# rbrito/deprecated-lame-mirror

Hardware: AMD Instinct MI355X
Metric: encoded audio seconds/sec (x real-time) at 44.1kHz stereo CBR128 (higher is better)
Workload: dtype f32

## Files before the change

### deprecated-lame-mirror_amd/csrc/lh_analysis.hip

```cpp
#include <stdint.h>
#include <math.h>

#ifdef LH_EMU
#include "hipemu.h"
#define LH_CONST static const
#else
#include <hip/hip_runtime.h>
#define LH_CONST __device__ static const
#endif

#if defined(LH_APROF) && !defined(LH_EMU)
__shared__ unsigned long long *lh_ap_base;
#define LH_PT(var) unsigned long long var = clock64()
#define LH_PA(idx, var) do { if (c.lane == 0) atomicAdd(&lh_ap_base[LH_NPROF * c.wave + 20 + (idx)], clock64() - var); } while (0)
#define LH_PC(idx) do { } while (0)
#endif
#define LH_CUSTOM_LDS "lh_lds_analysis.h"
#define LH_CUSTOM_SMP
#define LH_FZ_X(i) ((((i) >> 4) & 2) | (((i) >> 3) & 24) | (((i) >> 5) & 4))
#define LH_FZ(i) ((i) ^ LH_FZ_X(i))
#define LH_STAGE_IDX(i) LH_FZ(i)
#include "lh_static_tables.h"
#include "lh_dev_common.h"
#if !defined(LH_EMU)
// ... 312 lines not shown
    int     al[4], ah[4];
    if (K1 == 4) {
        int const x = LH_FZ_X(lo);
#pragma unroll
        for (int j = 0; j < 4; j++) {
            al[j] = (lo + j * K1) ^ x;
            ah[j] = (hi + j * K1) ^ x;
        }
    }
    else if (K1 == 16) {
        int const x = LH_FZ_X(blk * k4);
#pragma unroll
        for (int j = 0; j < 4; j++) {
            al[j] = (lo + j * K1) ^ x ^ (j >= 2 ? 2 : 0);
            ah[j] = (hi + j * K1) ^ x ^ (j >= 2 ? 2 : 0);
        }
    }
    else if (K1 == 64) {
#pragma unroll
        for (int j = 0; j < 4; j++) {
            al[j] = (lo + j * K1) ^ LH_FZ_X(64 * j);
            ah[j] = (hi + j * K1) ^ (2 ^ LH_FZ_X(64 * j));
        }
    }
    else {
        int const xl = LH_FZ_X(lo), xh = LH_FZ_X(hi);
#pragma unroll
        for (int j = 0; j < 4; j++) {
            al[j] = (lo + j * K1) ^ xl;
            ah[j] = (hi + j * K1) ^ xh;
        }
    }
    float const p0 = fz[al[0]], p1 = fz[al[1]], p2 = fz[al[2]], p3 = fz[al[3]];
    float const q0 = fz[ah[0]], q1 = fz[ah[1]], q2 = fz[ah[2]], q3 = fz[ah[3]];
    float const s01 = p0 + p1, d01 = p0 - p1, s23 = p2 + p3, d23 = p2 - p3;
    float const r2 = (float) (LH_SQRT2 * q2), r3 = (float) (LH_SQRT2 * q3);
    float const t01 = q0 + q1, u01 = q0 - q1;
    float const a_l0 = s01 + s23, a_l1 = d01 + d23, a_l2 = s01 - s23, a_l3 = d01 - d23;
    float const a_h0 = t01 + r2, a_h1 = u01 + r3, a_h2 = t01 - r2, a_h3 = u01 - r3;
    LhRot const rq1 = lh_rot(tw.z, tw.w, p1, q1);
    LhRot const rq3 = lh_rot(tw.z, tw.w, p3, q3);
    float const le = p0 + rq1.along, lm = p0 - rq1.along;
    float const he = q0 + rq1.across, hm = q0 - rq1.across;
    float const l2e = p2 + rq3.along, l2m = p2 - rq3.along;
    float const h2e = q2 + rq3.across, h2m = q2 - rq3.across;
    LhRot const ra = lh_rot(tw.x, tw.y, l2e, h2m);
    LhRot const rb = lh_rot(tw.y, tw.x, h2e, l2m);
    fz[al[0]] = axis ? a_l0 : le + ra.along;
    fz[al[1]] = axis ? a_l1 : lm + rb.across;
    fz[al[2]] = axis ? a_l2 : le - ra.along;
    fz[al[3]] = axis ? a_l3 : lm - rb.across;
    fz[ah[0]] = axis ? a_h0 : he + rb.along;
    fz[ah[1]] = axis ? a_h1 : hm + ra.across;
    fz[ah[2]] = axis ? a_h2 : he - rb.along;
    fz[ah[3]] = axis ? a_h3 : hm - ra.across;
}

LH_DEVFN void
lh_fft_long_inplace(const LhCtx & c, float *x)
{
    const float *w = c.T->fft_window;
    int const lane = c.lane;
    float   o[2][8];
#pragma unroll
    for (int q = 0; q < 2; q++) {
        int const jj = lane + 64 * q;
        int const i = (int) lh_rev8((unsigned) jj);
        const float *xs = x + (i ^ LH_FZ_X(i));
        float   f0, f1, f2, f3, ww;
        f0 = w[i] * xs[0];
        ww = w[i + 0x200] * xs[0x200];
        f1 = f0 - ww;
        f0 = f0 + ww;
        f2 = w[i + 0x100] * xs[0x100];
        ww = w[i + 0x300] * xs[0x300];
        f3 = f2 - ww;
        f2 = f2 + ww;
        o[q][0] = f0 + f2;
        o[q][2] = f0 - f2;
        o[q][1] = f1 + f3;
        o[q][3] = f1 - f3;
        f0 = w[i + 0x001] * xs[0x001];
        ww = w[i + 0x201] * xs[0x201];
        f1 = f0 - ww;
        f0 = f0 + ww;
        f2 = w[i + 0x101] * xs[0x101];
        ww = w[i + 0x301] * xs[0x301];
        f3 = f2 - ww;
        f2 = f2 + ww;
        o[q][4] = f0 + f2;
        o[q][6] = f0 - f2;
        o[q][5] = f1 + f3;
        o[q][7] = f1 - f3;
    }
    {
        lh_f32x4 tw[4][2];
#pragma unroll
        for (int stage = 0; stage < 4; stage++) {
            int const kx = 2 << (2 * stage);
#pragma unroll
            for (int q = 0; q < 2; q++)
                tw[stage][q] = *(const lh_f32x4 *) c.T->fht_tw[stage][(lane + 64 * q) % kx];
        }
        LH_WAVE_SYNC_MEM();
#pragma unroll
        for (int q = 0; q < 2; q++) {
            int const at = 4 * (lane + 64 * q), xa = LH_FZ_X(at);
#pragma unroll
            for (int k = 0; k < 4; k++) {
                x[(at + k) ^ xa] = o[q][k];
                x[(at + k + LH_BLKSIZE / 2) ^ xa] = o[q][4 + k];
            }
        }
        LH_WAVE_SYNC_MEM();
#pragma unroll
        for (int q = 0; q < 2; q++)
            lh_fht_unit_fz < 4 > (tw[0][q], x, lane + 64 * q);
        LH_WAVE_SYNC_MEM();
#pragma unroll
        for (int q = 0; q < 2; q++)
            lh_fht_unit_fz < 16 > (tw[1][q], x, lane + 64 * q);
        LH_WAVE_SYNC_MEM();
#pragma unroll
        for (int q = 0; q < 2; q++)
            lh_fht_unit_fz < 64 > (tw[2][q], x, lane + 64 * q);
        LH_WAVE_SYNC_MEM();
#pragma unroll
        for (int q = 0; q < 2; q++)
            lh_fht_unit_fz < 256 > (tw[3][q], x, lane + 64 * q);
        LH_WAVE_SYNC_MEM();
    }
}

LH_DEVFN void
lh_fft_short_inplace(const LhCtx & c, float *x)
{
    const float *ws = c.T->fft_window_s;
    int const lane = c.lane;
    float   o[2][8];
#pragma unroll
    for (int q = 0; q < 2; q++) {
        int const t = lane + 64 * q, tt = t < 3 * (LH_BLKSIZE_S / 8) ? t : 0;
        int const b = tt >> 5, j = tt & 31;
        int const k = (576 / 3) * (b + 1);
        int const i = (int) lh_rev8((unsigned) (j << 2));
        float   f0, f1, f2, f3, w;
        f0 = ws[i] * x[LH_FZ(i + k)];
        w = ws[0x7f - i] * x[LH_FZ(i + k + 0x80)];
        f1 = f0 - w;
        f0 = f0 + w;
        f2 = ws[i + 0x40] * x[LH_FZ(i + k + 0x40)];
        w = ws[0x3f - i] * x[LH_FZ(i + k + 0xc0)];
        f3 = f2 - w;
        f2 = f2 + w;
        o[q][0] = f0 + f2;
        o[q][2] = f0 - f2;
        o[q][1] = f1 + f3;
        o[q][3] = f1 - f3;
        f0 = ws[i + 0x01] * x[LH_FZ(i + k + 0x01)];
        w = ws[0x7e - i] * x[LH_FZ(i + k + 0x81)];
        f1 = f0 - w;
        f0 = f0 + w;
        f2 = ws[i + 0x41] * x[LH_FZ(i + k + 0x41)];
        w = ws[0x3e - i] * x[LH_FZ(i + k + 0xc1)];
        f3 = f2 - w;
        f2 = f2 + w;
        o[q][4] = f0 + f2;
        o[q][6] = f0 - f2;
        o[q][5] = f1 + f3;
        o[q][7] = f1 - f3;
    }
    LH_WAVE_SYNC_MEM();
#pragma unroll
    for (int q = 0; q < 2; q++) {
        int const t = lane + 64 * q;
        if (t < 3 * (LH_BLKSIZE_S / 8)) {
            int const at = (t >> 5) * LH_BLKSIZE_S + 4 * (t & 31);
#pragma unroll
            for (int k = 0; k < 4; k++) {
                x[LH_FZ(at + k)] = o[q][k];
                x[LH_FZ(at + k + LH_BLKSIZE_S / 2)] = o[q][4 + k];
            }
        }
    }
    LH_WAVE_SYNC_MEM();
    for (int t = lane; t < 3 * (LH_BLKSIZE_S / 8); t += 64) {
        int const b = t >> 5, u = t & 31;
        lh_fht_unit_fz < 4 > (*(const lh_f32x4 *) c.T->fht_tw[0][u % 2], x + b * LH_BLKSIZE_S, u);
    }
    LH_WAVE_SYNC_MEM();
    for (int t = lane; t < 3 * (LH_BLKSIZE_S / 8); t += 64) {
        int const b = t >> 5, u = t & 31;
        lh_fht_unit_fz < 16 > (*(const lh_f32x4 *) c.T->fht_tw[1][u % 8], x + b * LH_BLKSIZE_S, u);
    }
    LH_WAVE_SYNC_MEM();
    for (int t = lane; t < 3 * (LH_BLKSIZE_S / 8); t += 64) {
        int const b = t >> 5, u = t & 31;
        lh_fht_unit_fz < 64 > (*(const lh_f32x4 *) c.T->fht_tw[2][u % 32], x + b * LH_BLKSIZE_S, u);
    }
    LH_WAVE_SYNC_MEM();
}

LH_DEVFN void
lh_an_spectra_short(const LhCtx & c, int w, int both, const float *wl, const float *wr, int first, float *out_own, float *out_ms)
{
    float const sqrt2_half = (float) (LH_SQRT2 * 0.5f);
    int const n = LH_BLKSIZE_S, h = n >> 1;
    for (int m = c.lane; m <= h; m += 64) {
        int const ire = first + m, iim = first + ((m == 0) ? 0 : (n - m));
        float const lre = wl[LH_FZ(ire)], lim = wl[LH_FZ(iim)], rre = wr[LH_FZ(ire)], rim = wr[LH_FZ(iim)];
        float const ore = w ? rre : lre, oim = w ? rim : lim;
        float const mre = (w ? lre - rre : lre + rre) * sqrt2_half, mim = (w ? lim - rim : lim + rim) * sqrt2_half;
        out_own[m] = (m == 0) ? ore * ore : (ore * ore + oim * oim) * 0.5f;
        if (both)
            out_ms[m] = (m == 0) ? mre * mre : (mre * mre + mim * mim) * 0.5f;
    }
}

LH_DEVFN void
lh_an_spectra(const LhCtx & c, int w, int own, int ms, float *work)
{
    float const sqrt2_half = (float) (LH_SQRT2 * 0.5f);
    const float *wl = work, *wr = work + LH_BLKSIZE;
    float   eo[9], em[9];
#pragma unroll
    for (int k = 0; k < 9; k++) {
        int const m0 = c.lane + 64 * k, m = m0 <= LH_BLKSIZE / 2 ? m0 : LH_BLKSIZE / 2;
        int const ire = m, iim = (m == 0) ? 0 : (LH_BLKSIZE - m);
        float const lre = wl[LH_FZ(ire)], lim = wl[LH_FZ(iim)], rre = wr[LH_FZ(ire)], rim = wr[LH_FZ(iim)];
        float const ore = w ? rre : lre, oim = w ? rim : lim;
        float const mre = (w ? lre - rre : lre + rre) * sqrt2_half, mim = (w ? lim - rim : lim + rim) * sqrt2_half;
        eo[k] = (m == 0) ? ore * ore : (ore * ore + oim * oim) * 0.5f;
        em[k] = (m == 0) ? mre * mre : (mre * mre + mim * mim) * 0.5f;
    }
    LH_SYNC_WG_LDS();
#pragma unroll
    for (int k = 0; k < 9; k++) {
        int const m = c.lane + 64 * k;
        if (m <= LH_BLKSIZE / 2) {
            if (own)
                work[w * LH_AN_ROW + m] = eo[k];
            if (ms)
                work[(w + 2) * LH_AN_ROW + m] = em[k];
        }
    }
}

#ifndef LH_EMU
extern "C" __global__ void __launch_bounds__(LH_NT, 6)
#else
void
#endif
lh_analysis_kernel(const LhConfig * LH_KRESTRICT cfg, const LhTables * LH_KRESTRICT T, const int16_t * LH_KRESTRICT pcm, const float *pcmf, const LhStreamDesc * descs,
                   LhMidFrame * frames, int nstreams, LhStreamState * states)
{
#if defined(LH_APROF) && !defined(LH_EMU)
    unsigned long long *aprof = &states[blockIdx.y].prof[0][0];
    if (threadIdx.x == 0)
        lh_ap_base = aprof;
#endif
    LH_AP_T0();
    LhLds & L = lh_lds;
    LhLds & P = L;
    float  *const work = L.work;
#define LH_AN_E(chn) (work + (chn) * LH_AN_ROW)
    int const sidx = (int) blockIdx.y;
    LhCtx   c;
    c.cfg = cfg;
    c.T = T;
    c.st = nullptr;
    c.pcm = pcm;
    c.pcmf = pcmf;
    c.d = lh_desc_uniform(descs, sidx);
    c.tid = (int) threadIdx.x;
    c.lane = c.tid & 63;
    c.wave = lh_uni_i(c.tid >> 6);
    LhGranuleAt const ga = lh_granule_at(c.d, (int) blockIdx.x);
    if (!ga.live)
        return;
    int const lane = c.lane, w = c.wave, gr = ga.gr;
    int const n_chn_psy = (cfg->mode == LH_MODE_JOINT_STEREO) ? 4 : cfg->channels;
    int const bufbase = 576 + gr * 576 - LH_FFTOFFSET;
    LhMidGr *mg = &frames[ga.at].small.gr[gr];
    if (c.tid < 2)
        L.uselong[c.tid] = mg->uselong[c.tid];
    LH_AP(0);
    lh_stage_span < LH_BLKSIZE, LH_NT > (c, LH_SPAN, LH_SPAN + LH_BLKSIZE, ga.frame_base + bufbase);
    LH_SYNC_WG_LDS();
    LH_AP(1);
    if (w < cfg->channels)
        lh_fft_long_inplace(c, work + w * LH_BLKSIZE);
    LH_SYNC_WG_LDS();
    LH_AP(2);
    lh_an_spectra(c, w, w < n_chn_psy, n_chn_psy == 4, work);
    LH_WAVE_SYNC_MEM();
    const float *stg_s3 = T->psy_l.s3;
    LH_WAVE_SYNC_MEM();
    LH_AP(3);
    LH_AP(4);
    {
        int const chn = (lane == 1) ? w + 2 : w;
        int const summing = lane < 3 && chn < n_chn_psy;
        int const loud = (lane == 2);
        float  *prod = (w == 0) ? P.eb : P.thr;
        const float *ew = T->ath_eql_w;
        const float *e = LH_AN_E(summing ? chn : w);
        float   acc = 0.0f;
        for (int h = 0; h < 2; h++) {
            int const j0 = 256 * h;
            LH_WAVE_SYNC_MEM();
#pragma unroll
            for (int q = 0; q < 4; q++) {
                int const j = j0 + lane + 64 * q;
                prod[j - j0] = LH_AN_E(w)[j] * ew[j];
            }
            LH_WAVE_SYNC_MEM();
            if (summing) {
                const lh_f32x4 *s4 = (const lh_f32x4 *) ((loud ? prod - j0 : e) + j0);
                lh_f32x4 a0 = s4[0], a1 = s4[1], a2 = s4[2], a3 = s4[3];
                if (h == 0 && !loud) {
                    a0.x = a0.y = a0.z = a0.w = 0.0f;
                    a1.x = a1.y = a1.z = a1.w = 0.0f;
                    a2.x = a2.y = a2.z = 0.0f;
                }
                for (int g = 0; g < 64; g += 4) {
                    int const n = (g + 4 < 64) ? g + 4 : g;
                    lh_f32x4 const b0 = s4[n], b1 = s4[n + 1], b2 = s4[n + 2], b3 = s4[n + 3];
#ifndef LH_EMU
                    asm volatile("v_add_f32 %0, %0, %1\n\tv_add_f32 %0, %0, %2\n\tv_add_f32 %0, %0, %3\n\tv_add_f32 %0, %0, %4\n\t"
                                 "v_add_f32 %0, %0, %5\n\tv_add_f32 %0, %0, %6\n\tv_add_f32 %0, %0, %7\n\tv_add_f32 %0, %0, %8\n\t"
                                 "v_add_f32 %0, %0, %9\n\tv_add_f32 %0, %0, %10\n\tv_add_f32 %0, %0, %11\n\tv_add_f32 %0, %0, %12\n\t"
                                 "v_add_f32 %0, %0, %13\n\tv_add_f32 %0, %0, %14\n\tv_add_f32 %0, %0, %15\n\tv_add_f32 %0, %0, %16"
                                 : "+v"(acc)
                                 : "v"(a0.x), "v"(a0.y), "v"(a0.z), "v"(a0.w), "v"(a1.x), "v"(a1.y), "v"(a1.z), "v"(a1.w),
                                   "v"(a2.x), "v"(a2.y), "v"(a2.z), "v"(a2.w), "v"(a3.x), "v"(a3.y), "v"(a3.z), "v"(a3.w));
#else
                    acc += a0.x; acc += a0.y; acc += a0.z; acc += a0.w;
                    acc += a1.x; acc += a1.y; acc += a1.z; acc += a1.w;
                    acc += a2.x; acc += a2.y; acc += a2.z; acc += a2.w;
                    acc += a3.x; acc += a3.y; acc += a3.z; acc += a3.w;
#endif
                    a0 = b0;
                    a1 = b1;
                    a2 = b2;
                    a3 = b3;
                }
            }
        }
        if (summing) {
            if (!loud) {
                acc += e[LH_BLKSIZE / 2];
                mg->tot_ener[chn] = acc;
            }
            else {
                acc = (float) (acc * LH_VO_SCALE);
                mg->loud[w] = acc;
            }
        }
        LH_WAVE_SYNC_MEM();
    }
    LH_SYNC_WG_LDS();
    LH_AP(5);
    {
        LhMidLong *ml = &frames[ga.at].lng;
        if (n_chn_psy == 4) {
            LhMaskChan const two[2] = {
                {w, LH_AN_E(w), &P.eb[w * 64], &P.thr[w * 64], nullptr, nullptr, &ml->m[gr][w]},
                {w + 2, LH_AN_E(w + 2), &P.eb[(w + 2) * 64], &P.thr[(w + 2) * 64], nullptr, nullptr, &ml->m[gr][w + 2]}
            };
            lh_compute_masking < 2, 1 > (c, 1, two, stg_s3);
        }
        else if (w < n_chn_psy) {
            LhMaskChan const one[1] = { {w, LH_AN_E(w), &P.eb[w * 64], &P.thr[w * 64], nullptr, nullptr, &ml->m[gr][w]} };
            lh_compute_masking < 1, 1 > (c, 1, one, stg_s3);
        }
    }
    LH_AP(6);
    int const any_short = lh_uni_i(!(L.uselong[0] && L.uselong[1]));
    if (!any_short)
        return;
    LH_SYNC_WG_LDS();
    lh_stage_span < LH_BLKSIZE, LH_NT > (c, LH_SPAN, LH_SPAN + LH_BLKSIZE, ga.frame_base + bufbase);
    LH_SYNC_WG_LDS();
    if (!L.uselong[w])
        lh_fft_short_inplace(c, work + w * LH_BLKSIZE);
    LH_SYNC_WG_LDS();
    for (int sblock = 0; sblock < 3; sblock++) {
        if (w < n_chn_psy && !L.uselong[w]) {
            LhMidShort *ms = &frames[ga.at].shrt;
            int const both = (n_chn_psy == 4);
            lh_an_spectra_short(c, w, both, work, work + LH_BLKSIZE, sblock * LH_BLKSIZE_S, L.eshort[w], L.eshort[w + 2 < 4 ? w + 2 : 3]);
            LH_WAVE_SYNC_MEM();
            if (both) {
                LhMaskChan const two[2] = {
                    {w, L.eshort[w], &P.eb[w * 64], &P.thr[w * 64], nullptr, nullptr, &ms->m[gr][sblock][w]},
                    {w + 2, L.eshort[w + 2], &P.eb[(w + 2) * 64], &P.thr[(w + 2) * 64], nullptr, nullptr, &ms->m[gr][sblock][w + 2]}
                };
                lh_compute_masking < 2, 1 > (c, 0, two, T->psy_s.s3);
            }
            else {
                LhMaskChan const one[1] = { {w, L.eshort[w], &P.eb[w * 64], &P.thr[w * 64], nullptr, nullptr, &ms->m[gr][sblock][w]} };
                lh_compute_masking < 1, 1 > (c, 0, one, T->psy_s.s3);
            }
        }
        LH_SYNC_WG_LDS();
    }
    LH_AP(7);
}

#ifndef LH_EMU
extern "C" int
lh_launch_analysis(const LhConfig * cfg, const LhTables * T, const int16_t * pcm, const float *pcmf, const LhStreamDesc * descs,
                   const LhStreamState * states, LhMidPools mid, int nstreams, int max_frames, void *stream)
{
    if (nstreams <= 0 || max_frames <= 0)
        return 0;
    dim3 const grid((unsigned) (LH_NGR * max_frames), (unsigned) nstreams);
    hipLaunchKernelGGL(lh_attack_kernel, grid, dim3(64), 0, (hipStream_t) stream, cfg, pcm, pcmf, descs, mid.frames, nstreams);
    hipLaunchKernelGGL(lh_attack_scan_kernel, dim3((unsigned) nstreams), dim3(64), 0, (hipStream_t) stream, cfg, T, descs, states,
                       mid.frames, nstreams);
    hipLaunchKernelGGL(lh_analysis_kernel, grid, dim3(LH_NT), 0, (hipStream_t) stream, cfg, T, pcm, pcmf, descs, mid.frames, nstreams,
                       (LhStreamState *) states);
    return (int) hipGetLastError();
}
#else
extern "C" int
lh_emu_analysis(const LhConfig * cfg, const LhTables * T, const int16_t * pcm, const float *pcmf, const LhStreamDesc * descs,
                const LhStreamState * states, const LhMidPools * pools, int nstreams, int max_frames)
{
    LhMidPools const mid = *pools;
    hipemu_dim3 grid = { (unsigned) (LH_NGR * max_frames), (unsigned) nstreams, 1 }, b64 = { 64, 1, 1 }, b128 = { LH_NT, 1, 1 };
    hipemu_dim3 grid1 = { (unsigned) nstreams, 1, 1 };
    hipemu_run(grid, b64,[=] () {
               lh_attack_kernel(cfg, pcm, pcmf, descs, mid.frames, nstreams);
               }
    );
    hipemu_run(grid1, b64,[=] () {
               lh_attack_scan_kernel(cfg, T, descs, states, mid.frames, nstreams);
               }
    );
    hipemu_run(grid, b128,[=] () {
               lh_analysis_kernel(cfg, T, pcm, pcmf, descs, mid.frames, nstreams, (LhStreamState *) states);
               }
    );
    return 0;
}
#endif
```

### deprecated-lame-mirror_amd/csrc/lh_dev_psy_core.h

```cpp
#ifndef LH_DEV_PSY_CORE_H
#define LH_DEV_PSY_CORE_H

#include "lh_dev_common.h"

#define LH_NSFIRLEN 21
#define LH_RPELEV  2
#define LH_RPELEV2 16
#define LH_PREECHO_ATT0 0.8
#define LH_PREECHO_ATT1 0.6
#define LH_PREECHO_ATT2 0.3
#define LH_VO_SCALE (1./( 14752*14752 )/(LH_BLKSIZE/2))

LH_DEVCONST float lh_psy_tab[9] = {
    1.0f, 0.79433f, 0.63096f, 0.63096f, 0.63096f, 0.63096f, 0.63096f, 0.25119f, 0.11749f
};
LH_DEVCONST int lh_mask_add_delta[9] = { 2, 2, 2, 1, 1, 1, 0, 0, -1 };
LH_DEVFN float
lh_psy_tab_at(int i)
{
    return (i == 0) ? 1.0f : (i == 1) ? 0.79433f : (i < 7) ? 0.63096f : (i == 7) ? 0.25119f : 0.11749f;
}

LH_DEVFN int
lh_mask_add_delta_at(int i)
// ... 138 lines not shown
    }
    {
        lh_f32x4 tw[4][2];
#pragma unroll
        for (int stage = 0; stage < 4; stage++) {
            int const kx = 2 << (2 * stage);
#pragma unroll
            for (int q = 0; q < 2; q++)
                tw[stage][q] = *(const lh_f32x4 *) c.T->fht_tw[stage][(lane + 64 * q) % kx];
        }
        LH_WAVE_SYNC_MEM();
#pragma unroll
        for (int stage = 0; stage < 4; stage++) {
            int const k1 = 4 << (2 * stage);
#pragma unroll
            for (int q = 0; q < 2; q++)
                lh_fht_unit(tw[stage][q], x, k1, lane + 64 * q);
            LH_WAVE_SYNC_MEM();
        }
    }
}

LH_DEVFN void
lh_fft_short(const LhCtx & c, int ch, int base, float *x)
{
    const float *ws = c.T->fft_window_s;
    int     lane = c.lane;
    for (int t = lane; t < 3 * (LH_BLKSIZE_S / 8); t += 64) {
        int const b = t >> 5, j = t & 31;
        int const k = (576 / 3) * (b + 1) + base;
        float   f0, f1, f2, f3, w;
        float  *o = x + b * LH_BLKSIZE_S + 4 * j;
        int     i = (int) lh_rev8((unsigned) (j << 2));
        f0 = ws[i] * lh_smp(c, ch, i + k);
        w = ws[0x7f - i] * lh_smp(c, ch, i + k + 0x80);
        f1 = f0 - w;
        f0 = f0 + w;
        f2 = ws[i + 0x40] * lh_smp(c, ch, i + k + 0x40);
        w = ws[0x3f - i] * lh_smp(c, ch, i + k + 0xc0);
        f3 = f2 - w;
        f2 = f2 + w;
        o[0] = f0 + f2;
        o[2] = f0 - f2;
        o[1] = f1 + f3;
        o[3] = f1 - f3;
        f0 = ws[i + 0x01] * lh_smp(c, ch, i + k + 0x01);
        w = ws[0x7e - i] * lh_smp(c, ch, i + k + 0x81);
        f1 = f0 - w;
        f0 = f0 + w;
        f2 = ws[i + 0x41] * lh_smp(c, ch, i + k + 0x41);
        w = ws[0x3e - i] * lh_smp(c, ch, i + k + 0xc1);
        f3 = f2 - w;
        f2 = f2 + w;
        o[LH_BLKSIZE_S / 2 + 0] = f0 + f2;
        o[LH_BLKSIZE_S / 2 + 2] = f0 - f2;
        o[LH_BLKSIZE_S / 2 + 1] = f1 + f3;
        o[LH_BLKSIZE_S / 2 + 3] = f1 - f3;
    }
    LH_WAVE_SYNC_MEM();
    for (int stage = 0, k1 = 4; stage < 3; stage++, k1 <<= 2) {
        for (int t = lane; t < 3 * (LH_BLKSIZE_S / 8); t += 64) {
            int const b = t >> 5, u = t & 31;
            lh_f32x4 const tw = *(const lh_f32x4 *) c.T->fht_tw[stage][u % (k1 >> 1)];
            lh_fht_unit(tw, x + b * LH_BLKSIZE_S, k1, u);
        }
        LH_WAVE_SYNC_MEM();
    }
}

LH_DEVFN void
lh_fft_energy(const LhCtx & c, int chn, const float *wl, const float *wr, int n, float *out)
{
    float const sqrt2_half = (float) (LH_SQRT2 * 0.5f);
    int const h = n >> 1;
    for (int m = c.lane; m <= h; m += 64) {
        int const ire = m, iim = (m == 0) ? 0 : (n - m);
        float   re, im;
        if (chn == 0) {
            re = wl[ire];
            im = wl[iim];
        }
        else if (chn == 1) {
            re = wr[ire];
            im = wr[iim];
        }
        else if (chn == 2) {
            re = (wl[ire] + wr[ire]) * sqrt2_half;
            im = (wl[iim] + wr[iim]) * sqrt2_half;
        }
        else {
            re = (wl[ire] - wr[ire]) * sqrt2_half;
            im = (wl[iim] - wr[iim]) * sqrt2_half;
        }
        if (m == 0)
            out[0] = re * re;
        else
            out[m] = (re * re + im * im) * 0.5f;
    }
}

LH_DEVFN void
lh_fft_energy_pair(const LhCtx & c, int w, const float *wl, const float *wr, int n, float *out_own, float *out_ms)
{
    float const sqrt2_half = (float) (LH_SQRT2 * 0.5f);
    int const h = n >> 1;
    for (int m = c.lane; m <= h; m += 64) {
        int const ire = m, iim = (m == 0) ? 0 : (n - m);
        float const lre = wl[ire], lim = wl[iim], rre = wr[ire], rim = wr[iim];
        float const ore = w ? rre : lre, oim = w ? rim : lim;
        float const mre = (w ? lre - rre : lre + rre) * sqrt2_half, mim = (w ? lim - rim : lim + rim) * sqrt2_half;
        out_own[m] = (m == 0) ? ore * ore : (ore * ore + oim * oim) * 0.5f;
        out_ms[m] = (m == 0) ? mre * mre : (mre * mre + mim * mim) * 0.5f;
    }
}

LH_DEVFN void
lh_partition2sfb_wave(LhPsyBand const *gd, float const *eb, float const *thr, float *enn_out,
                      float *thm_out, int out_stride, float thm_scale, int replicate3, int lane,
                      int active)
{
    int const npart = gd->npart;
    int const n_sb = gd->n_sb;
    int const sb = lane;
    float   enn = 0.0f, thmm = 0.0f, tv;
    int     b, live, m;
    {
        int const bo_k = gd->bo[lane < n_sb ? lane : 0];
        int const d = (bo_k < npart ? bo_k : npart) - lane;
        uint32_t const run = lh_wave_scan_max_u32((lane < n_sb && d > 0) ? (uint32_t) d : 0u);
        uint32_t const prev = lh_shfl_u32(run, (lane - 1) & 63);
        m = lane > 0 ? (int) prev : 0;
    }
    LH_WAVE_SYNC_MEM();
    b = sb + m;
    live = (sb == 0) || (b - 1 < npart);
    if (!active || sb >= n_sb)
        return;
    if (live) {
        int const bo_sb = gd->bo[sb];
        int const b_lim = bo_sb < npart ? bo_sb : npart;
        if (sb > 0) {
            float const carry_w = 1.0f - gd->bo_weight[sb - 1];
            enn = carry_w * eb[b - 1];
            thmm = carry_w * thr[b - 1];
        }
        while (b < b_lim) {
            enn += eb[b];
            thmm += thr[b];
            b++;
        }
        if (b < npart) {
            float const w_curr = gd->bo_weight[sb];
            enn += w_curr * eb[b];
            thmm += w_curr * thr[b];
        }
        tv = thm_scale < 0 ? thmm : thmm * thm_scale;
    }
    else {
        enn = 0;
        tv = thm_scale < 0 ? 0.0f : 0.0f * thm_scale;
    }
    enn_out[sb * out_stride] = enn;
    thm_out[sb * out_stride] = tv;
    if (replicate3) {
        enn_out[sb * out_stride + 1] = enn_out[sb * out_stride + 2] = enn;
        thm_out[sb * out_stride + 1] = thm_out[sb * out_stride + 2] = tv;
    }
}

struct LhSfbChan {
    const float *eb, *thr;
    float  *en, *thm;
};

template < int NC > LH_DEVFN void
lh_partition2sfb_long(const LhTables * T, const LhSfbChan (&ch)[NC], int lane)
{
    int const est = lane >= 32;
    int const sb = est ? lane - 32 : lane;
    LhPsyBand const *gd = est ? &T->psy_l_to_s : &T->psy_l;
    int const npart = gd->npart;
    int const n_sb = est ? T->psy_l_to_s.n_sb : T->psy_l.n_sb;
    int const mine = sb < n_sb;
    int const sbc = mine ? sb : 0;
    int const bo_sb = gd->bo[sbc];
    float const w_prev = gd->bo_weight[sbc > 0 ? sbc - 1 : 0], w_curr = gd->bo_weight[sbc];
    int const b_lim = bo_sb < npart ? bo_sb : npart;
    int     m;
    {
        int const d = b_lim - sb;
        uint32_t const v = (mine && d > 0) ? (uint32_t) d : 0u;
        uint32_t const run_l = lh_wave_scan_max_u32(est ? 0u : v);
        uint32_t const run_e = lh_wave_scan_max_u32((est && lane >= 32) ? v : 0u);
        uint32_t const run = est ? run_e : run_l;
        uint32_t const prev = lh_shfl_u32(run, (lane - 1) & 63);
        m = (sb > 0) ? (int) prev : 0;
    }
    LH_WAVE_SYNC_MEM();
    {
        int const b0 = sb + m;
        int const live = (sb == 0) || (b0 - 1 < npart);
        int const steps = (mine && live && b_lim > b0) ? b_lim - b0 : 0;
        int const nmax = lh_uni_i((int) lh_wave_max_u32((uint32_t) steps));
        int const bend = b0 + steps;
        float   enn[NC], thmm[NC];
#pragma unroll
        for (int q = 0; q < NC; q++) {
            int const carry = mine && live && sb > 0;
            float const cw = 1.0f - w_prev;
            float const e = ch[q].eb[carry ? b0 - 1 : 0], t = ch[q].thr[carry ? b0 - 1 : 0];
            enn[q] = carry ? cw * e : 0.0f;
            thmm[q] = carry ? cw * t : 0.0f;
        }
        for (int i = 0; i < nmax; i++) {
            int const on = i < steps;
            int const b = on ? b0 + i : 0;
#pragma unroll
            for (int q = 0; q < NC; q++) {
                float const e = ch[q].eb[b], t = ch[q].thr[b];
                float const se = enn[q] + e, st = thmm[q] + t;
                enn[q] = on ? se : enn[q];
                thmm[q] = on ? st : thmm[q];
            }
        }
        {
            int const tail = mine && live && bend < npart;
#pragma unroll
            for (int q = 0; q < NC; q++) {
                float const e = ch[q].eb[tail ? bend : 0], t = ch[q].thr[tail ? bend : 0];
                float const se = enn[q] + w_curr * e, st = thmm[q] + w_curr * t;
                float   ev, tv;
                enn[q] = tail ? se : enn[q];
                thmm[q] = tail ? st : thmm[q];
                ev = live ? enn[q] : 0.0f;
                tv = live ? thmm[q] : 0.0f;
                if (est)
                    tv = tv * (float) (1. / 64.f);
                if (mine) {
                    if (est) {
                        ch[q].en[22 + 3 * sb] = ch[q].en[22 + 3 * sb + 1] = ch[q].en[22 + 3 * sb + 2] = ev;
                        ch[q].thm[22 + 3 * sb] = ch[q].thm[22 + 3 * sb + 1] = ch[q].thm[22 + 3 * sb + 2] = tv;
                    }
                    else {
                        ch[q].en[sb] = ev;
                        ch[q].thm[sb] = tv;
                    }
                }
            }
        }
    }
}

LH_DEVFN int
lh_mask_index(LhPsyBand const *gd, int b, float m0, float m1, float m2, float a0, float a1, float a2)
{
    float   m, a;
    int     k, nl;
    int const np = gd->npart;
    if (b == 0) {
        a = a1 + a2;
        m = m1;
        if (m < m2)
            m = m2;
        nl = gd->numlines[0] + gd->numlines[1] - 1;
        if (!(a > 0.0f))
            return 0;
        a = 20.0f * (m * 2.0f - a) / (a * nl);
    }
    else if (b == np - 1) {
        a = a0 + a1;
        m = m0;
        if (m < m1)
            m = m1;
        nl = gd->numlines[b - 1] + gd->numlines[b] - 1;
        if (!(a > 0.0f))
            return 0;
        a = 20.0f * (m * 2.0f - a) / (a * nl);
    }
    else {
        a = a0 + a1 + a2;
        m = m0;
        if (m < m1)
            m = m1;
        if (m < m2)
            m = m2;
        nl = gd->numlines[b - 1] + gd->numlines[b] + gd->numlines[b + 1] - 1;
        if (!(a > 0.0f))
            return 0;
        a = 20.0f * (m * 3.0f - a) / (a * nl);
    }
    k = (int) a;
    if (k > 8)
        k = 8;
    return k;
}

LH_DEVFN float
lh_mask_add_far(float m1, float m2, double bound)
{
    float const hi = __builtin_fmaxf(m1, m2), lo = __builtin_fminf(m1, m2);
    return ((double) hi < bound * (double) lo) ? m1 + m2 : hi;
}

struct LhMaskChan {
    int     chn;
    const float *energy;
    float  *eb, *thr;
    float  *nb1, *nb2;
    LhMidMask *raw;
};


template < int NC, int FRONT = 0 > LH_DEVFN void
lh_compute_masking(const LhCtx & c, int is_long, const LhMaskChan (&ch)[NC], const float *s3)
{
    double  mid[10];
#pragma unroll
    for (int j = 0; j < 10; j++)
        mid[j] = lh_uni_f64(c.T->mask_mid[j]);
    double const far_bound = mid[9];
    LhPsyBand const *gd = is_long ? &c.T->psy_l : &c.T->psy_s;
    int const b = c.lane;
    int const np = gd->npart;
    int const on = b < np;
    int const bc = on ? b : 0;
    int const t_numlines = gd->numlines[bc], t_first = gd->s3ind[bc][0], t_last = gd->s3ind[bc][1], t_row = gd->s3_row[bc];
    float const t_rnum = gd->rnumlines[bc], t_mlow = gd->masking_lower[bc], t_minval = gd->minval[bc];
    float   ebb[NC], m[NC], avg[NC], th[NC], ecb[NC];
    int     tone[NC], delta[NC], dd[NC];
    LH_PT(t_mk);
#pragma unroll
    for (int q = 0; q < NC; q++)
        ebb[q] = m[q] = th[q] = ecb[q] = 0;
    {
        int const n = on ? t_numlines : 0;
        int const j0 = (int) lh_wave_scan_u32((uint32_t) n) - n;
        float const rn = on ? t_rnum : 0.0f;
        int const nmax = lh_uni_i((int) lh_wave_max_u32((uint32_t) n));
#if !defined(LH_EMU)
        float   nx[NC][8];
#pragma unroll
        for (int q = 0; q < NC; q++)
#pragma unroll
            for (int u = 0; u < 8; u++)
                nx[q][u] = ch[q].energy[j0 + u];
        for (int i = 0; i < nmax; i += 8) {
            int const rem = n - i;
            float   cu[NC][8];
#pragma unroll
            for (int q = 0; q < NC; q++)
#pragma unroll
                for (int u = 0; u < 8; u++) {
                    cu[q][u] = nx[q][u];
                    nx[q][u] = ch[q].energy[j0 + i + 8 + u];
                }
#pragma unroll
            for (int q = 0; q < NC; q++) {
                float const a0 = cu[q][0], a1 = cu[q][1], a2 = cu[q][2], a3 = cu[q][3], a4 = cu[q][4], a5 = cu[q][5], a6 = cu[q][6], a7 = cu[q][7];
                unsigned long long sv, tm;
#define LH_PS_TERM(K, A) "v_cmpx_gt_i32_e64 %[tm], %[rem], " #K "\n\tv_add_f32 %[eb], %[eb], %[" #A "]\n\tv_max_f32 %[mx], %[mx], %[" #A "]\n\t"
                asm volatile("s_mov_b64 %[sv], exec\n\t"
                             LH_PS_TERM(0, a0) LH_PS_TERM(1, a1) LH_PS_TERM(2, a2) LH_PS_TERM(3, a3)
                             LH_PS_TERM(4, a4) LH_PS_TERM(5, a5) LH_PS_TERM(6, a6) LH_PS_TERM(7, a7)
                             "s_mov_b64 exec, %[sv]"
                             : [eb] "+v"(ebb[q]), [mx] "+v"(m[q]), [sv] "=&s"(sv), [tm] "=&s"(tm)
                             : [rem] "v"(rem), [a0] "v"(a0), [a1] "v"(a1), [a2] "v"(a2), [a3] "v"(a3),
                               [a4] "v"(a4), [a5] "v"(a5), [a6] "v"(a6), [a7] "v"(a7));
#undef LH_PS_TERM
            }
        }
#else
        for (int i = 0; i < nmax; i += 8) {
            float   el[NC][8];
#pragma unroll
            for (int q = 0; q < NC; q++)
#pragma unroll
                for (int u = 0; u < 8; u++)
                    el[q][u] = ch[q].energy[j0 + ((i + u < n) ? i + u : 0)];
#pragma unroll
            for (int u = 0; u < 8; u++)
#pragma unroll
                for (int q = 0; q < NC; q++) {
                    float const e = (i + u < n) ? el[q][u] : 0.0f;
                    ebb[q] += e;
                    m[q] = __builtin_fmaxf(m[q], e);
                }
        }
#endif
#pragma unroll
        for (int q = 0; q < NC; q++) {
            avg[q] = ebb[q] * rn;
            ch[q].eb[b] = ebb[q];
        }
    }
    LH_PA(14, t_mk);
    {
        int const lo = (b > 0) ? b - 1 : 0, hi = (b < 63) ? b + 1 : 63;
#pragma unroll
        for (int q = 0; q < NC; q++) {
            float const m0 = lh_shfl_f32(m[q], lo), m2 = lh_shfl_f32(m[q], hi);
            float const a0 = lh_shfl_f32(avg[q], lo), a2 = lh_shfl_f32(avg[q], hi);
            tone[q] = on ? lh_mask_index(gd, b, m0, m[q], m2, a0, avg[q], a2) : 0;
            ch[q].thr[b] = lh_psy_tab_at(tone[q]);
            delta[q] = lh_mask_add_delta_at(tone[q]);
        }
    }
    int const first = on ? t_first : 1, last = on ? t_last : 0;
    int const krel = (on ? t_row : 0) - first;
    int     n1, n3;
    {
        uint32_t t[2];
#pragma unroll
        for (int q = 0; q < NC; q++) {
            uint32_t const P = lh_wave_scan_u32((uint32_t) tone[q]);
            uint32_t const pl = lh_shfl_u32(P, last & 63), pf = lh_shfl_u32(P, (first - 1) & 63);
            dd[q] = (int) (pl - ((first > 0) ? pf : 0u));
        }
        t[0] = (uint32_t) ((on && b - 3 - first > 0) ? b - 3 - first : 0);
        t[1] = (uint32_t) ((on && last - b - 2 > 0) ? last - b - 2 : 0);
        lh_wave_max_n < 2 > (t);
        n1 = lh_uni_i((int) t[0]);
        n3 = lh_uni_i((int) t[1]);
    }
    LH_WAVE_SYNC_MEM();
    LH_PA(15, t_mk);
#define LH_SPREAD_X(q_, kk_) (s3[krel + (kk_)] * ch[q_].eb[(kk_)] * ch[q_].thr[(kk_)])
#pragma unroll
    for (int q = 0; q < NC; q++)
        ecb[q] = on ? LH_SPREAD_X(q, first) : 0.0f;
    {
        int     kk = b - 2 - n1;
        int     act = kk > first && kk <= last;
        float   x[NC];
#pragma unroll
        for (int q = 0; q < NC; q++)
            x[q] = LH_SPREAD_X(q, act ? kk : first);
        for (int j = 0; j < n1; j++) {
            int const act_n = (kk + 1 > first) && (kk + 1 <= last) && (j + 1 < n1);
            int const kn = act_n ? kk + 1 : first;
#pragma unroll
            for (int q = 0; q < NC; q++) {
                float const xn = LH_SPREAD_X(q, kn);
                float const r = lh_mask_add_far(ecb[q], x[q], far_bound);
                ecb[q] = act ? r : ecb[q];
                x[q] = xn;
            }
            act = act_n;
            ++kk;
        }
    }
    for (int j = 0; j < 5; j++) {
        int const kk = b - 2 + j;
        int const act = kk > first && kk <= last;
        int const d = (j < 2) ? 2 - j : j - 2;
        int const kc = act ? kk : first;
#pragma unroll
        for (int q = 0; q < NC; q++) {
            int const near = act && d <= delta[q];
            float const x = LH_SPREAD_X(q, kc);
            float   r = lh_mask_add_far(ecb[q], x, far_bound);
            if (lh_ballot(near)) {
                float const rn = lh_mask_add_near(mid, ecb[q], x);
                r = near ? rn : r;
            }
            ecb[q] = act ? r : ecb[q];
        }
    }
    {
        int     kk = b + 3;
        int     act = kk > first && kk <= last;
        float   x[NC];
#pragma unroll
        for (int q = 0; q < NC; q++)
            x[q] = LH_SPREAD_X(q, act ? kk : first);
        for (int j = 0; j < n3; j++) {
            int const act_n = (kk + 1 > first) && (kk + 1 <= last);
            int const kn = act_n ? kk + 1 : first;
#pragma unroll
            for (int q = 0; q < NC; q++) {
                float const xn = LH_SPREAD_X(q, kn);
                float const r = lh_mask_add_far(ecb[q], x[q], far_bound);
                ecb[q] = act ? r : ecb[q];
                x[q] = xn;
            }
            act = act_n;
            ++kk;
        }
    }
#undef LH_SPREAD_X
    LH_PA(16, t_mk);
    if (FRONT) {
        int const dd_n = last - first + 1;
#pragma unroll
        for (int q = 0; q < NC; q++) {
            int const di = on ? (1 + 2 * dd[q]) / (2 * dd_n) : 0;
            float const avg_mask = lh_psy_tab_at(di) * 0.5f;
            float   e = ecb[q], x = m[q];
            e *= avg_mask;
            x *= t_minval;
            x *= avg_mask;
            ch[q].raw->v[0][b] = ebb[q];
            ch[q].raw->v[1][b] = on ? e : 0.0f;
            ch[q].raw->v[2][b] = on ? x : 0.0f;
        }
        LH_WAVE_SYNC_MEM();
        return;
    }
    if (on) {
        float const masking_lower = t_mlow * lh_lds.ss.masking_lower;
        int const dd_n = last - first + 1;
#pragma unroll
        for (int q = 0; q < NC; q++) {
            float   x, avg_mask, e = ecb[q], t;
            int const di = (1 + 2 * dd[q]) / (2 * dd_n);
            avg_mask = lh_psy_tab_at(di) * 0.5f;
            e *= avg_mask;
            if (is_long) {
                int const bt_old = lh_lds.ss.blocktype_old[ch[q].chn & 1];
                float const n1v = *ch[q].nb1, n2v = *ch[q].nb2;
                if (bt_old == LH_SHORT_TYPE) {
                    float const ecb_limit = LH_RPELEV * n1v;
                    if (ecb_limit > 0)
                        t = __builtin_fminf(e, ecb_limit);
                    else {
                        float const alt = (float) (ebb[q] * LH_PREECHO_ATT2);
                        t = __builtin_fminf(e, alt);
                    }
                }
                else {
                    float   lim2 = LH_RPELEV2 * n2v;
                    float   lim1 = LH_RPELEV * n1v;
                    float   lim;
                    if (lim2 <= 0)
                        lim2 = e;
                    if (lim1 <= 0)
                        lim1 = e;
                    if (bt_old == LH_NORM_TYPE)
                        lim = __builtin_fminf(lim1, lim2);
                    else
                        lim = lim1;
                    t = __builtin_fminf(e, lim);
                }
                *ch[q].nb2 = n1v;
                *ch[q].nb1 = e;
            }
            else
                t = e;
            x = m[q];
            x *= t_minval;
            x *= avg_mask;
            if (t > x)
                t = x;
            if (masking_lower > 1)
                t *= masking_lower;
            if (t > ebb[q])
                t = ebb[q];
            if (masking_lower < 1)
                t *= masking_lower;
            th[q] = t;
        }
    }
    LH_WAVE_SYNC_MEM();
#pragma unroll
    for (int q = 0; q < NC; q++)
        ch[q].thr[b] = th[q];
    LH_WAVE_SYNC_MEM();
    LH_PA(17, t_mk);
}

#endif
```

### deprecated-lame-mirror_amd/csrc/lh_lds_analysis.h

```cpp
#define LH_AN_ROW (LH_HBLKSIZE + 3)
struct LhLds {
    LhSmallState ss;
    LhCtxShared ctx;
    LhRgSlot rg[2];
    int     uselong[2];
    int     pad[2];
    float   work[4 * LH_AN_ROW] __attribute__((aligned(16)));
    float   eshort[4][LH_HBLKSIZE_S + 3] __attribute__((aligned(16)));
    float   eb[4 * 64];
    float   thr[4 * 64];
};
static_assert(4 * LH_AN_ROW >= 2 * LH_BLKSIZE, "both channels' spans fit the spectra's place");
__shared__ LhLds lh_lds __attribute__((aligned(16)));
```

Measured before the change: 85270.

## Interleave eb/thr into paired LDS array and restructure partition-sum loads

Merges the separate per-channel eb and thr LDS arrays into one interleaved array so the spreading loop fetches both values with a single 8-byte LDS read. For the FRONT masking path, the partition energy summation is rewritten to alternate loads between the two channels (or two halves for a single channel), guarding loads by remaining count, so loads overlap the asm accumulation. The loudness product scratch buffer is moved into the new array. This adds code-path divergence between FRONT and non-FRONT variants and relies on correct aliasing of the scratch region.

```diff
diff --git a/deprecated-lame-mirror_amd/csrc/lh_analysis.hip b/deprecated-lame-mirror_amd/csrc/lh_analysis.hip
--- a/deprecated-lame-mirror_amd/csrc/lh_analysis.hip
+++ b/deprecated-lame-mirror_amd/csrc/lh_analysis.hip
@@ -638,7 +638,7 @@
         int const chn = (lane == 1) ? w + 2 : w;
         int const summing = lane < 3 && chn < n_chn_psy;
         int const loud = (lane == 2);
-        float  *prod = (w == 0) ? P.eb : P.thr;
+        float  *prod = P.ebt + 256 * w;
         const float *ew = T->ath_eql_w;
         const float *e = LH_AN_E(summing ? chn : w);
         float   acc = 0.0f;
@@ -701,13 +701,13 @@
         LhMidLong *ml = &frames[ga.at].lng;
         if (n_chn_psy == 4) {
             LhMaskChan const two[2] = {
-                {w, LH_AN_E(w), &P.eb[w * 64], &P.thr[w * 64], nullptr, nullptr, &ml->m[gr][w]},
-                {w + 2, LH_AN_E(w + 2), &P.eb[(w + 2) * 64], &P.thr[(w + 2) * 64], nullptr, nullptr, &ml->m[gr][w + 2]}
+                {w, LH_AN_E(w), &P.ebt[w * 128], nullptr, nullptr, nullptr, &ml->m[gr][w]},
+                {w + 2, LH_AN_E(w + 2), &P.ebt[(w + 2) * 128], nullptr, nullptr, nullptr, &ml->m[gr][w + 2]}
             };
             lh_compute_masking < 2, 1 > (c, 1, two, stg_s3);
         }
         else if (w < n_chn_psy) {
-            LhMaskChan const one[1] = { {w, LH_AN_E(w), &P.eb[w * 64], &P.thr[w * 64], nullptr, nullptr, &ml->m[gr][w]} };
+            LhMaskChan const one[1] = { {w, LH_AN_E(w), &P.ebt[w * 128], nullptr, nullptr, nullptr, &ml->m[gr][w]} };
             lh_compute_masking < 1, 1 > (c, 1, one, stg_s3);
         }
     }
@@ -729,13 +729,13 @@
             LH_WAVE_SYNC_MEM();
             if (both) {
                 LhMaskChan const two[2] = {
-                    {w, L.eshort[w], &P.eb[w * 64], &P.thr[w * 64], nullptr, nullptr, &ms->m[gr][sblock][w]},
-                    {w + 2, L.eshort[w + 2], &P.eb[(w + 2) * 64], &P.thr[(w + 2) * 64], nullptr, nullptr, &ms->m[gr][sblock][w + 2]}
+                    {w, L.eshort[w], &P.ebt[w * 128], nullptr, nullptr, nullptr, &ms->m[gr][sblock][w]},
+                    {w + 2, L.eshort[w + 2], &P.ebt[(w + 2) * 128], nullptr, nullptr, nullptr, &ms->m[gr][sblock][w + 2]}
                 };
                 lh_compute_masking < 2, 1 > (c, 0, two, T->psy_s.s3);
             }
             else {
-                LhMaskChan const one[1] = { {w, L.eshort[w], &P.eb[w * 64], &P.thr[w * 64], nullptr, nullptr, &ms->m[gr][sblock][w]} };
+                LhMaskChan const one[1] = { {w, L.eshort[w], &P.ebt[w * 128], nullptr, nullptr, nullptr, &ms->m[gr][sblock][w]} };
                 lh_compute_masking < 1, 1 > (c, 0, one, T->psy_s.s3);
             }
         }
diff --git a/deprecated-lame-mirror_amd/csrc/lh_dev_psy_core.h b/deprecated-lame-mirror_amd/csrc/lh_dev_psy_core.h
--- a/deprecated-lame-mirror_amd/csrc/lh_dev_psy_core.h
+++ b/deprecated-lame-mirror_amd/csrc/lh_dev_psy_core.h
@@ -464,6 +464,29 @@
     return ((double) hi < bound * (double) lo) ? m1 + m2 : hi;
 }
 
+#if !defined(LH_EMU)
+#define LH_PS_TERM(K, A) "v_cmpx_gt_i32_e64 %[tm], %[rem], " #K "\n\tv_add_f32 %[eb], %[eb], %[" #A "]\n\tv_max_f32 %[mx], %[mx], %[" #A "]\n\t"
+LH_DEVFN void
+lh_partition_terms(float &eb, float &mx, int rem, const float (&a)[8])
+{
+    unsigned long long sv, tm;
+    asm volatile("s_mov_b64 %[sv], exec\n\t"
+                 LH_PS_TERM(0, a0) LH_PS_TERM(1, a1) LH_PS_TERM(2, a2) LH_PS_TERM(3, a3)
+                 LH_PS_TERM(4, a4) LH_PS_TERM(5, a5) LH_PS_TERM(6, a6) LH_PS_TERM(7, a7)
+                 "s_mov_b64 exec, %[sv]"
+                 : [eb] "+v"(eb), [mx] "+v"(mx), [sv] "=&s"(sv), [tm] "=&s"(tm)
+                 : [rem] "v"(rem), [a0] "v"(a[0]), [a1] "v"(a[1]), [a2] "v"(a[2]), [a3] "v"(a[3]),
+                   [a4] "v"(a[4]), [a5] "v"(a[5]), [a6] "v"(a[6]), [a7] "v"(a[7]));
+}
+#endif
+
+LH_DEVFN float
+lh_spread_pair(float s, const float *pairs, int kk)
+{
+    lh_f32x2 const p = ((const lh_f32x2 *) pairs)[kk];
+    return s * p.x * p.y;
+}
+
 struct LhMaskChan {
     int     chn;
     const float *energy;
@@ -500,37 +523,65 @@
         float const rn = on ? t_rnum : 0.0f;
         int const nmax = lh_uni_i((int) lh_wave_max_u32((uint32_t) n));
 #if !defined(LH_EMU)
-        float   nx[NC][8];
-#pragma unroll
-        for (int q = 0; q < NC; q++)
+        if (FRONT) {
+            float   bx[8], by[8];
+            int     rem = n;
+            int const step = (NC == 2) ? 8 : 16, ofy = (NC == 2) ? 0 : 8;
+#define LH_PS_LOAD(R, Q, AT, MORE) \
+            if (rem > (MORE)) { \
+                _Pragma("unroll") for (int u = 0; u < 8; u++) \
+                    R[u] = ch[Q].energy[j0 + (AT) + u]; \
+            }
 #pragma unroll
             for (int u = 0; u < 8; u++)
-                nx[q][u] = ch[q].energy[j0 + u];
-        for (int i = 0; i < nmax; i += 8) {
-            int const rem = n - i;
-            float   cu[NC][8];
+                bx[u] = by[u] = 0.0f;
+            LH_PS_LOAD(bx, 0, 0, 0)
+            for (int i = 0; i < nmax; i += step) {
+                LH_PS_LOAD(by, NC - 1, i + ofy, ofy)
+                lh_partition_terms(ebb[0], m[0], rem, bx);
+                if (NC == 1) {
+                    rem -= 8;
+                    if (i + 8 >= nmax)
+                        break;
+                }
+                LH_PS_LOAD(bx, 0, i + step, 8)
+                lh_partition_terms(ebb[NC - 1], m[NC - 1], rem, by);
+                rem -= 8;
+            }
+#undef LH_PS_LOAD
+        }
+        else {
+            float   nx[NC][8];
 #pragma unroll
             for (int q = 0; q < NC; q++)
 #pragma unroll
-                for (int u = 0; u < 8; u++) {
-                    cu[q][u] = nx[q][u];
-                    nx[q][u] = ch[q].energy[j0 + i + 8 + u];
+                for (int u = 0; u < 8; u++)
+                    nx[q][u] = ch[q].energy[j0 + u];
+            for (int i = 0; i < nmax; i += 8) {
+                int const rem = n - i;
+                float   cu[NC][8];
+#pragma unroll
+                for (int q = 0; q < NC; q++)
+#pragma unroll
+                    for (int u = 0; u < 8; u++) {
+                        cu[q][u] = nx[q][u];
+                        nx[q][u] = ch[q].energy[j0 + i + 8 + u];
+                    }
+#pragma unroll
+                for (int q = 0; q < NC; q++) {
+                    float const a0 = cu[q][0], a1 = cu[q][1], a2 = cu[q][2], a3 = cu[q][3], a4 = cu[q][4], a5 = cu[q][5], a6 = cu[q][6], a7 = cu[q][7];
+                    unsigned long long sv, tm;
+                    asm volatile("s_mov_b64 %[sv], exec\n\t"
+                                 LH_PS_TERM(0, a0) LH_PS_TERM(1, a1) LH_PS_TERM(2, a2) LH_PS_TERM(3, a3)
+                                 LH_PS_TERM(4, a4) LH_PS_TERM(5, a5) LH_PS_TERM(6, a6) LH_PS_TERM(7, a7)
+                                 "s_mov_b64 exec, %[sv]"
+                                 : [eb] "+v"(ebb[q]), [mx] "+v"(m[q]), [sv] "=&s"(sv), [tm] "=&s"(tm)
+                                 : [rem] "v"(rem), [a0] "v"(a0), [a1] "v"(a1), [a2] "v"(a2), [a3] "v"(a3),
+                                   [a4] "v"(a4), [a5] "v"(a5), [a6] "v"(a6), [a7] "v"(a7));
                 }
-#pragma unroll
-            for (int q = 0; q < NC; q++) {
-                float const a0 = cu[q][0], a1 = cu[q][1], a2 = cu[q][2], a3 = cu[q][3], a4 = cu[q][4], a5 = cu[q][5], a6 = cu[q][6], a7 = cu[q][7];
-                unsigned long long sv, tm;
-#define LH_PS_TERM(K, A) "v_cmpx_gt_i32_e64 %[tm], %[rem], " #K "\n\tv_add_f32 %[eb], %[eb], %[" #A "]\n\tv_max_f32 %[mx], %[mx], %[" #A "]\n\t"
-                asm volatile("s_mov_b64 %[sv], exec\n\t"
-                             LH_PS_TERM(0, a0) LH_PS_TERM(1, a1) LH_PS_TERM(2, a2) LH_PS_TERM(3, a3)
-                             LH_PS_TERM(4, a4) LH_PS_TERM(5, a5) LH_PS_TERM(6, a6) LH_PS_TERM(7, a7)
-                             "s_mov_b64 exec, %[sv]"
-                             : [eb] "+v"(ebb[q]), [mx] "+v"(m[q]), [sv] "=&s"(sv), [tm] "=&s"(tm)
-                             : [rem] "v"(rem), [a0] "v"(a0), [a1] "v"(a1), [a2] "v"(a2), [a3] "v"(a3),
-                               [a4] "v"(a4), [a5] "v"(a5), [a6] "v"(a6), [a7] "v"(a7));
+            }
+        }
 #undef LH_PS_TERM
-            }
-        }
 #else
         for (int i = 0; i < nmax; i += 8) {
             float   el[NC][8];
@@ -552,7 +603,7 @@
 #pragma unroll
         for (int q = 0; q < NC; q++) {
             avg[q] = ebb[q] * rn;
-            ch[q].eb[b] = ebb[q];
+            ch[q].eb[FRONT ? 2 * b : b] = ebb[q];
         }
     }
     LH_PA(14, t_mk);
@@ -563,7 +614,10 @@
             float const m0 = lh_shfl_f32(m[q], lo), m2 = lh_shfl_f32(m[q], hi);
             float const a0 = lh_shfl_f32(avg[q], lo), a2 = lh_shfl_f32(avg[q], hi);
             tone[q] = on ? lh_mask_index(gd, b, m0, m[q], m2, a0, avg[q], a2) : 0;
-            ch[q].thr[b] = lh_psy_tab_at(tone[q]);
+            if (FRONT)
+                ch[q].eb[2 * b + 1] = lh_psy_tab_at(tone[q]);
+            else
+                ch[q].thr[b] = lh_psy_tab_at(tone[q]);
             delta[q] = lh_mask_add_delta_at(tone[q]);
         }
     }
@@ -586,7 +640,8 @@
     }
     LH_WAVE_SYNC_MEM();
     LH_PA(15, t_mk);
-#define LH_SPREAD_X(q_, kk_) (s3[krel + (kk_)] * ch[q_].eb[(kk_)] * ch[q_].thr[(kk_)])
+#define LH_SPREAD_X(q_, kk_) (FRONT ? lh_spread_pair(s3[krel + (kk_)], ch[q_].eb, (kk_)) \
+                                    : s3[krel + (kk_)] * ch[q_].eb[(kk_)] * ch[q_].thr[(kk_)])
 #pragma unroll
     for (int q = 0; q < NC; q++)
         ecb[q] = on ? LH_SPREAD_X(q, first) : 0.0f;
diff --git a/deprecated-lame-mirror_amd/csrc/lh_lds_analysis.h b/deprecated-lame-mirror_amd/csrc/lh_lds_analysis.h
--- a/deprecated-lame-mirror_amd/csrc/lh_lds_analysis.h
+++ b/deprecated-lame-mirror_amd/csrc/lh_lds_analysis.h
@@ -7,8 +7,7 @@
     int     pad[2];
     float   work[4 * LH_AN_ROW] __attribute__((aligned(16)));
     float   eshort[4][LH_HBLKSIZE_S + 3] __attribute__((aligned(16)));
-    float   eb[4 * 64];
-    float   thr[4 * 64];
+    float   ebt[4 * 128] __attribute__((aligned(16)));
 };
 static_assert(4 * LH_AN_ROW >= 2 * LH_BLKSIZE, "both channels' spans fit the spectra's place");
 __shared__ LhLds lh_lds __attribute__((aligned(16)));
```

After: 85620, median of 6. Within noise of the previous version (+0.4%).
